# selftok-team/SelftokTokenizer

Measured on NVIDIA B200. Metric: images/sec encode+50-step decode, 256x256/512-tok, higher is better.
Workload: dtype fp16 (IEEE-half operands on tcgen05, fp32 accumulate; encoder/VQ/tables fp32)

## Files before the change

selftoktokenizer_b200/build.py:

```python
from __future__ import annotations

import os
import subprocess
import sys
from concurrent.futures import ThreadPoolExecutor

CSRC = os.path.join(os.path.dirname(os.path.abspath(__file__)), "csrc")
LIB = os.path.join(CSRC, "libselftok_b200.so")
SOURCES = ["kernels_simt.cu", "gemm_tc.cu", "attn_tc5.cu", "engine.cu", "vae.cu"]
HEADERS = ["common.cuh", "kernels.h", os.path.join("..", "..", "include", "selftok_b200.h")]
NVCC_FLAGS = ["-gencode", "arch=compute_100a,code=sm_100a", "-O3", "-lineinfo", "-std=c++17",
              "-Xcompiler", "-fPIC", "-Xcompiler", "-fvisibility=hidden", "--expt-relaxed-constexpr"]


def _nvcc() -> str:
    for c in (os.environ.get("NVCC"), "/usr/local/cuda/bin/nvcc", "nvcc"):
        if c and (os.path.isabs(c) and os.path.exists(c) or not os.path.isabs(c)):
            return c
    raise RuntimeError("nvcc not found")


def needs_build() -> bool:
    if not os.path.exists(LIB):
        return True
    t = os.path.getmtime(LIB)
    deps = [os.path.join(CSRC, f) for f in SOURCES + HEADERS]
    return any(os.path.getmtime(d) > t for d in deps)


def build(force: bool = False, verbose: bool = False) -> str:
    if not force and not needs_build():
        return LIB
    nvcc = _nvcc()
# ... 27 lines not shown
```

selftoktokenizer_b200/csrc/attn_tc5.cu:

```cuda
#include "common.cuh"
#include "kernels.h"

#include <cuda.h>

#include <algorithm>
#include <cstdlib>

namespace stk {

int make_tensor_map_2d(CUtensorMap* map, const void* ptr, uint64_t rows, uint64_t cols, uint32_t box_rows, uint32_t box_cols,
                       int fp16);

namespace {

constexpr int HD = 64, BQ = 128, BKV = 64;
#ifndef SELFTOK_ATTN5_NSB
#define SELFTOK_ATTN5_NSB 2
#endif
constexpr int NSB = SELFTOK_ATTN5_NSB;
#ifndef SELFTOK_ATTN5_SPLIT_ISSUE
#define SELFTOK_ATTN5_SPLIT_ISSUE 0
#endif
constexpr bool SPLIT_ISSUE = SELFTOK_ATTN5_SPLIT_ISSUE != 0;
constexpr int Q_BYTES = BQ * HD * 2, KV_TILE_BYTES = BKV * HD * 2;
constexpr int XCH_BYTES = 6 * BQ * 4;
#ifndef SELFTOK_ATTN5_SPLIT_CTAS
#define SELFTOK_ATTN5_SPLIT_CTAS 2
#endif
template <int NSPLIT> struct A5 {
  static constexpr int PL = NSPLIT == 3 ? 2 : 1;
  static constexpr int MIN_CTAS = NSPLIT == 3 ? SELFTOK_ATTN5_SPLIT_CTAS : 2;
  static constexpr int KV_STAGES = NSPLIT == 3 ? (MIN_CTAS == 2 ? 2 : 3) : 4;
  static constexpr int Q_STAGES = (NSPLIT == 3 && MIN_CTAS == 2) ? 1 : 2;
  static constexpr int Q_STAGE = PL * Q_BYTES;
  static constexpr int KV_STAGE = PL * 2 * KV_TILE_BYTES;
  static constexpr int SMEM_TILES = Q_STAGES * Q_STAGE + KV_STAGES * KV_STAGE;
  static constexpr int SMEM_BYTES = SMEM_TILES + 1024 + 256 + XCH_BYTES;
};
constexpr int TMEM_COLS = 256;
constexpr int NUM_THREADS = 64 + 8 * 32;
constexpr float kRescaleThreshold = 8.0f;

__device__ __forceinline__ uint32_t smem_u32(const void* p) { return (uint32_t)__cvta_generic_to_shared(p); }
__device__ __forceinline__ void mbar_init(uint32_t bar, uint32_t count) {
  asm volatile("mbarrier.init.shared::cta.b64 [%0], %1;" ::"r"(bar), "r"(count) : "memory");
}
__device__ __forceinline__ void mbar_expect_tx(uint32_t bar, uint32_t bytes) {
  asm volatile("mbarrier.arrive.expect_tx.shared::cta.b64 _, [%0], %1;" ::"r"(bar), "r"(bytes) : "memory");
}
__device__ __forceinline__ void mbar_arrive(uint32_t bar) {
  asm volatile("mbarrier.arrive.shared::cta.b64 _, [%0];" ::"r"(bar) : "memory");
}
constexpr uint32_t kSuspendHintNs = 20000;
__device__ __forceinline__ bool mbar_try_wait(uint32_t bar, uint32_t parity) {
  uint32_t ok;
  asm volatile(
      "{\n\t.reg .pred p;\n\t"
      "mbarrier.try_wait.parity.shared::cta.b64 p, [%1], %2, %3;\n\t"
      "selp.u32 %0, 1, 0, p;\n\t}"
      : "=r"(ok) : "r"(bar), "r"(parity), "r"(kSuspendHintNs) : "memory");
  return ok != 0;
}
__device__ __forceinline__ bool mbar_test(uint32_t bar, uint32_t parity) {
  uint32_t ok;
  asm volatile(
      "{\n\t.reg .pred p;\n\t"
      "mbarrier.test_wait.parity.shared::cta.b64 p, [%1], %2;\n\t"
      "selp.u32 %0, 1, 0, p;\n\t}"
      : "=r"(ok) : "r"(bar), "r"(parity) : "memory");
  return ok != 0;
}
__device__ __forceinline__ void mbar_wait(uint32_t bar, uint32_t parity) {
  if (mbar_try_wait(bar, parity)) return;
  const long long t0 = clock64();
  uint32_t spins = 0;
  while (!mbar_try_wait(bar, parity)) {
    if ((++spins & 0x3ff) == 0 && clock64() - t0 > 8000000000LL) {
      printf("selftok attn_tc5: mbarrier timeout (block %d,%d,%d thread %d bar %u parity %u)\n", blockIdx.x, blockIdx.y, blockIdx.z,
             threadIdx.x, bar, parity);
      __trap();
    }
  }
}
__device__ __forceinline__ void tma_load_2d(uint32_t dst, const CUtensorMap* map, uint32_t bar, int c0, int c1) {
  asm volatile(
      "cp.async.bulk.tensor.2d.shared::cluster.global.mbarrier::complete_tx::bytes [%0], [%1, {%3, %4}], [%2];"
      ::"r"(dst), "l"(reinterpret_cast<uint64_t>(map)), "r"(bar), "r"(c0), "r"(c1) : "memory");
}
__device__ __forceinline__ void tc_fence_before() { asm volatile("tcgen05.fence::before_thread_sync;" ::: "memory"); }
__device__ __forceinline__ void tc_fence_after() { asm volatile("tcgen05.fence::after_thread_sync;" ::: "memory"); }
__device__ __forceinline__ void tc_commit(uint32_t bar) {
  asm volatile("tcgen05.commit.cta_group::1.mbarrier::arrive::one.shared::cluster.b64 [%0];" ::"r"(bar) : "memory");
}
__device__ __forceinline__ void tc_mma_f16(uint32_t d_tmem, uint64_t a_desc, uint64_t b_desc, uint32_t idesc, uint32_t accumulate) {
  asm volatile(
      "{\n\t.reg .pred p;\n\t"
      "setp.ne.b32 p, %4, 0;\n\t"
      "tcgen05.mma.cta_group::1.kind::f16 [%0], %1, %2, %3, p;\n\t}"
      ::"r"(d_tmem), "l"(a_desc), "l"(b_desc), "r"(idesc), "r"(accumulate) : "memory");
}
__device__ __forceinline__ void tc_mma_f16_ts(uint32_t d_tmem, uint32_t a_tmem, uint64_t b_desc, uint32_t idesc, uint32_t accumulate) {
  asm volatile(
      "{\n\t.reg .pred p;\n\t"
      "setp.ne.b32 p, %4, 0;\n\t"
      "tcgen05.mma.cta_group::1.kind::f16 [%0], [%1], %2, %3, p;\n\t}"
      ::"r"(d_tmem), "r"(a_tmem), "l"(b_desc), "r"(idesc), "r"(accumulate) : "memory");
}
__device__ __forceinline__ void tmem_ld32(uint32_t taddr, uint32_t (&r)[32]) {
  asm volatile(
      "tcgen05.ld.sync.aligned.32x32b.x32.b32 "
      "{%0, %1, %2, %3, %4, %5, %6, %7, %8, %9, %10, %11, %12, %13, %14, %15, "
      "%16, %17, %18, %19, %20, %21, %22, %23, %24, %25, %26, %27, %28, %29, %30, %31}, [%32];"
      : "=r"(r[0]), "=r"(r[1]), "=r"(r[2]), "=r"(r[3]), "=r"(r[4]), "=r"(r[5]), "=r"(r[6]), "=r"(r[7]),
        "=r"(r[8]), "=r"(r[9]), "=r"(r[10]), "=r"(r[11]), "=r"(r[12]), "=r"(r[13]), "=r"(r[14]), "=r"(r[15]),
        "=r"(r[16]), "=r"(r[17]), "=r"(r[18]), "=r"(r[19]), "=r"(r[20]), "=r"(r[21]), "=r"(r[22]), "=r"(r[23]),
        "=r"(r[24]), "=r"(r[25]), "=r"(r[26]), "=r"(r[27]), "=r"(r[28]), "=r"(r[29]), "=r"(r[30]), "=r"(r[31])
      : "r"(taddr) : "memory");
}
__device__ __forceinline__ void tmem_st32(uint32_t taddr, const uint32_t (&r)[32]) {
  asm volatile(
      "tcgen05.st.sync.aligned.32x32b.x32.b32 [%0], "
      "{%1, %2, %3, %4, %5, %6, %7, %8, %9, %10, %11, %12, %13, %14, %15, %16, "
      "%17, %18, %19, %20, %21, %22, %23, %24, %25, %26, %27, %28, %29, %30, %31, %32};"
      ::"r"(taddr), "r"(r[0]), "r"(r[1]), "r"(r[2]), "r"(r[3]), "r"(r[4]), "r"(r[5]), "r"(r[6]), "r"(r[7]),
        "r"(r[8]), "r"(r[9]), "r"(r[10]), "r"(r[11]), "r"(r[12]), "r"(r[13]), "r"(r[14]), "r"(r[15]),
        "r"(r[16]), "r"(r[17]), "r"(r[18]), "r"(r[19]), "r"(r[20]), "r"(r[21]), "r"(r[22]), "r"(r[23]),
        "r"(r[24]), "r"(r[25]), "r"(r[26]), "r"(r[27]), "r"(r[28]), "r"(r[29]), "r"(r[30]), "r"(r[31])
      : "memory");
}
__device__ __forceinline__ void tmem_st16(uint32_t taddr, const uint32_t (&r)[16]) {
  asm volatile(
      "tcgen05.st.sync.aligned.32x32b.x16.b32 [%0], "
      "{%1, %2, %3, %4, %5, %6, %7, %8, %9, %10, %11, %12, %13, %14, %15, %16};"
      ::"r"(taddr), "r"(r[0]), "r"(r[1]), "r"(r[2]), "r"(r[3]), "r"(r[4]), "r"(r[5]), "r"(r[6]), "r"(r[7]),
        "r"(r[8]), "r"(r[9]), "r"(r[10]), "r"(r[11]), "r"(r[12]), "r"(r[13]), "r"(r[14]), "r"(r[15])
      : "memory");
}
__device__ __forceinline__ void tmem_ld_wait() { asm volatile("tcgen05.wait::ld.sync.aligned;" ::: "memory"); }
__device__ __forceinline__ void tmem_st_wait() { asm volatile("tcgen05.wait::st.sync.aligned;" ::: "memory"); }

__device__ __forceinline__ uint64_t make_smem_desc(uint32_t smem_addr) {
  uint64_t d = 0;
  d |= (uint64_t)((smem_addr >> 4) & 0x3FFF);
  d |= (uint64_t)1 << 16;
  d |= (uint64_t)(1024 >> 4) << 32;
  d |= (uint64_t)1 << 46;
  d |= (uint64_t)2 << 61;
  return d;
}
__device__ __forceinline__ uint32_t make_idesc(int m, int n, int fp16, int b_mn_major) {
  const uint32_t fmt = fp16 ? 0u : 1u;
  return (1u << 4) | (fmt << 7) | (fmt << 10) | ((uint32_t)b_mn_major << 16) | ((uint32_t)(n >> 3) << 17) | ((uint32_t)(m >> 4) << 24);
}

__device__ __forceinline__ float ex2_approx(float x) {
  float y;
  asm("ex2.approx.ftz.f32 %0, %1;" : "=f"(y) : "f"(x));
  return y;
}
__device__ __forceinline__ void scale_sub2(uint32_t s0, uint32_t s1, float scale, float nsub, float& x0, float& x1) {
  asm("{\n\t.reg .b64 x, sc, sb;\n\t"
      "mov.b64 x, {%2, %3};\n\t"
      "mov.b64 sc, {%4, %4};\n\t"
      "mov.b64 sb, {%5, %5};\n\t"
      "fma.rn.f32x2 x, x, sc, sb;\n\t"
      "mov.b64 {%0, %1}, x;\n\t}"
      : "=f"(x0), "=f"(x1) : "r"(s0), "r"(s1), "f"(scale), "f"(nsub));
}
__device__ __forceinline__ void add2(float& a0, float& a1, float e0, float e1) {
  asm("{\n\t.reg .b64 a, b;\n\t"
      "mov.b64 a, {%0, %1};\n\t"
      "mov.b64 b, {%2, %3};\n\t"
      "add.f32x2 a, a, b;\n\t"
      "mov.b64 {%0, %1}, a;\n\t}"
      : "+f"(a0), "+f"(a1) : "f"(e0), "f"(e1));
}
__device__ __forceinline__ uint32_t pack2_16(float lo, float hi, bool fp16) {
  uint32_t r;
  if (fp16) asm("cvt.rn.f16x2.f32 %0, %1, %2;" : "=r"(r) : "f"(hi), "f"(lo));
  else asm("cvt.rn.bf16x2.f32 %0, %1, %2;" : "=r"(r) : "f"(hi), "f"(lo));
  return r;
}

struct Attn5Params {
  AttnOut out;
  int B, S, H, ctx_rows, ctx_keys, fp16;
  float scale_log2e;
};

template <bool FP16, int NSPLIT>
__global__ void __launch_bounds__(NUM_THREADS, A5<NSPLIT>::MIN_CTAS)
attention_tc5_kernel(const __grid_constant__ CUtensorMap map_q, const __grid_constant__ CUtensorMap map_kv,
                     const __grid_constant__ CUtensorMap map_q_lo, const __grid_constant__ CUtensorMap map_kv_lo, const Attn5Params p) {
  static_assert(NSPLIT == 1 || (NSPLIT == 3 && !FP16), "split mode uses bf16 planes");
  using C = A5<NSPLIT>;
  constexpr int KV_STAGES = C::KV_STAGES;
  extern __shared__ uint8_t smem_raw[];
  const uint32_t base = (smem_u32(smem_raw) + 1023u) & ~1023u;
  const uint32_t q_s = base;
  constexpr int QS = C::Q_STAGES;
  static_assert(!SPLIT_ISSUE || QS == 2, "the two-issuer experiment prefetches Q one item ahead");
  const uint32_t kv_s = base + QS * C::Q_STAGE;
  const uint32_t bars = kv_s + KV_STAGES * C::KV_STAGE;
  auto q_full = [&](int qb) { return bars + 8u * qb; };
  auto q_empty = [&](int qb) { return bars + 16 + 8u * qb; };
  auto p_ready = [&](int pb) { return bars + 32 + 8u * pb; };
// ... 282 lines not shown
      }
    }
    if (pend_item >= 0) epilogue(pend_item, n - 1, pend_g, pend_l);
  }
  tc_fence_before();
  __syncthreads();
  if (warp == 2) {
    tc_fence_after();
    asm volatile("tcgen05.dealloc.cta_group::1.sync.aligned.b32 %0, %1;" ::"r"(tmem_base), "r"((uint32_t)TMEM_COLS) : "memory");
  }
}

int g_num_sms_dev[64];
bool g_attr_dev[64];

}

int launch_attention_tc5(const __nv_bfloat16* qkv16, int B, int S, int H, int ctx_rows, int ctx_keys, const AttnOut& out,
                         cudaStream_t s, int fp16, const __nv_bfloat16* qkv_lo) {
  STK_CHECK(qkv16 && B > 0 && S > 0 && H > 0, -1, "attention_tc5: bad arguments");
  STK_CHECK(out.ld % 8 == 0, -1, "attention_tc5: output pitch must be a multiple of 8");
  STK_CHECK(ctx_keys <= S && ctx_rows <= S && ctx_keys >= 0 && ctx_rows >= 0, -1, "attention_tc5: context limits exceed the sequence");
  STK_CHECK(!(fp16 && qkv_lo), -1, "attention_tc5: the split mode uses bf16 planes");
  STK_TRY(gemm_tc_init());
  int dev = 0;
  STK_CUDA(cudaGetDevice(&dev));
  STK_CHECK(dev >= 0 && dev < 64, -1, "attention_tc5: device ordinal out of range");
  if (!g_attr_dev[dev]) {
    STK_CUDA(cudaDeviceGetAttribute(&g_num_sms_dev[dev], cudaDevAttrMultiProcessorCount, dev));
    STK_CUDA(cudaFuncSetAttribute(attention_tc5_kernel<true, 1>, cudaFuncAttributeMaxDynamicSharedMemorySize, A5<1>::SMEM_BYTES));
    STK_CUDA(cudaFuncSetAttribute(attention_tc5_kernel<false, 1>, cudaFuncAttributeMaxDynamicSharedMemorySize, A5<1>::SMEM_BYTES));
    STK_CUDA(cudaFuncSetAttribute(attention_tc5_kernel<false, 3>, cudaFuncAttributeMaxDynamicSharedMemorySize, A5<3>::SMEM_BYTES));
    g_attr_dev[dev] = true;
  }
  const int g_num_sms = g_num_sms_dev[dev];
  CUtensorMap mq, mkv, mql, mkvl;
  const uint64_t rows = (uint64_t)B * S, cols = (uint64_t)3 * H * HD;
  STK_TRY(make_tensor_map_2d(&mq, qkv16, rows, cols, BQ, HD, fp16));
  STK_TRY(make_tensor_map_2d(&mkv, qkv16, rows, cols, BKV, HD, fp16));
  mql = mq; mkvl = mkv;
  if (qkv_lo) {
    STK_TRY(make_tensor_map_2d(&mql, qkv_lo, rows, cols, BQ, HD, 0));
    STK_TRY(make_tensor_map_2d(&mkvl, qkv_lo, rows, cols, BKV, HD, 0));
  }
  Attn5Params p{out, B, S, H, ctx_rows, ctx_keys, fp16, 0.125f * 1.4426950408889634f};
  const int n_items = ((S + BQ - 1) / BQ) * H * B;
  if (qkv_lo) {
    dim3 grid(std::min(n_items, A5<3>::MIN_CTAS * g_num_sms));
    attention_tc5_kernel<false, 3><<<grid, NUM_THREADS, A5<3>::SMEM_BYTES, s>>>(mq, mkv, mql, mkvl, p);
  } else {
    static const int ctas_per_sm = [] { const char* e = getenv("SELFTOK_ATTN5_CTAS_PER_SM"); return (e && e[0] == '1') ? 1 : 2; }();
    dim3 grid(std::min(n_items, ctas_per_sm * g_num_sms));
    if (fp16) attention_tc5_kernel<true, 1><<<grid, NUM_THREADS, A5<1>::SMEM_BYTES, s>>>(mq, mkv, mql, mkvl, p);
    else attention_tc5_kernel<false, 1><<<grid, NUM_THREADS, A5<1>::SMEM_BYTES, s>>>(mq, mkv, mql, mkvl, p);
  }
  count_launch();
  STK_CUDA(cudaGetLastError());
  return 0;
}

}
```

selftoktokenizer_b200/csrc/kernels.h:

```cpp
#pragma once
#include <cuda_runtime.h>
#include <cuda_bf16.h>
#include <stdint.h>

namespace stk {

enum EpiMode { EPI_STORE = 0, EPI_RESID = 1, EPI_SPLIT = 2 };
struct Epilogue {
  int mode = EPI_STORE;
  int act = 0;
  const float* bias = nullptr;
  float* out = nullptr;
  int64_t ldo = 0;
  const float* resid = nullptr;
  const float* gate = nullptr;
  int64_t gate_ld = 0;
  int gate_period = 1;
  const float* addtab = nullptr;
  int64_t add_ld = 0;
  int add_period = 1;
  __nv_bfloat16* out_hi = nullptr;
  __nv_bfloat16* out_lo = nullptr;
  int rpb_in = 0, rpb_out = 0, row_off = 0;
  int fp16 = 0;
// ... 36 lines not shown
int launch_unpatchify_axpy(const float* o, const float* x_in, float* x_out, float dt, int B, int C, int g, int p,
                           cudaStream_t s, const float* o_u = nullptr, float cfg_scale = 1.f);
int launch_transpose(const float* in, float* out, int rows, int cols, cudaStream_t s);
int launch_split_bf16(const float* in, __nv_bfloat16* hi, __nv_bfloat16* lo, int64_t n, cudaStream_t s, int fp16 = 0);
int launch_bcast_rows(const float* src, const float* add, float* out, int B, int64_t rows, int64_t cols, cudaStream_t s);
int launch_crop_pos(const float* pos, float* out, int max_size, int g, int D, cudaStream_t s);
int launch_copy_rows(const float* src, int64_t src_bs, float* dst, int64_t dst_bs, int B, int64_t n_per_batch, cudaStream_t s);

int launch_gemm_tc(const __nv_bfloat16* A_hi, const __nv_bfloat16* A_lo, const __nv_bfloat16* W_hi,
                   const __nv_bfloat16* W_lo, int64_t M, int N, int K, int nsplit, const Epilogue& ep,
                   cudaStream_t s, int fp16 = 0);
struct TcProblem {
  const __nv_bfloat16* A_hi; const __nv_bfloat16* A_lo; const __nv_bfloat16* W_hi; const __nv_bfloat16* W_lo;
  int64_t M; int N; int K;
  Epilogue ep;
  int conv_C = 0, conv_H = 0, conv_W = 0, conv_stride = 1;
};
int launch_gemm_tc_grouped(const TcProblem* probs, int n, int nsplit, cudaStream_t s, int fp16 = 0);
int gemm_tc_init();
void gemm_tc_set_ctas(int n);

int launch_attention_tc5(const __nv_bfloat16* qkv16, int B, int S, int H, int ctx_rows, int ctx_keys, const AttnOut& out,
                         cudaStream_t s, int fp16, const __nv_bfloat16* qkv_lo = nullptr);

}
```

Measured before the change: 21.25.

## Add persistent ping-pong attention kernel with 128-key tiles for non-split path

Adds a new persistent tcgen05 attention kernel that runs two softmax warpgroups in ping-pong over paired query tiles, with 128-wide KV tiles, a 3-stage KV pipeline and a full 512-column TMEM allocation. The single-plane fp16/bf16 path now dispatches to it, and the old NSPLIT=1 variant is dropped. Shared device helpers move into a common header. The aim is to overlap QK/PV MMAs with softmax and to reuse each K/V load across two query tiles, at the cost of one CTA per SM and more complex barrier scheduling.

```diff
diff --git a/selftoktokenizer_b200/build.py b/selftoktokenizer_b200/build.py
--- a/selftoktokenizer_b200/build.py
+++ b/selftoktokenizer_b200/build.py
@@ -7,8 +7,8 @@
 
 CSRC = os.path.join(os.path.dirname(os.path.abspath(__file__)), "csrc")
 LIB = os.path.join(CSRC, "libselftok_b200.so")
-SOURCES = ["kernels_simt.cu", "gemm_tc.cu", "attn_tc5.cu", "engine.cu", "vae.cu"]
-HEADERS = ["common.cuh", "kernels.h", os.path.join("..", "..", "include", "selftok_b200.h")]
+SOURCES = ["kernels_simt.cu", "gemm_tc.cu", "attn_tc5.cu", "attn_pp.cu", "engine.cu", "vae.cu"]
+HEADERS = ["common.cuh", "attn_common.cuh", "kernels.h", os.path.join("..", "..", "include", "selftok_b200.h")]
 NVCC_FLAGS = ["-gencode", "arch=compute_100a,code=sm_100a", "-O3", "-lineinfo", "-std=c++17",
               "-Xcompiler", "-fPIC", "-Xcompiler", "-fvisibility=hidden", "--expt-relaxed-constexpr"]
 
diff --git a/selftoktokenizer_b200/csrc/attn_common.cuh b/selftoktokenizer_b200/csrc/attn_common.cuh
--- /dev/null
+++ b/selftoktokenizer_b200/csrc/attn_common.cuh
@@ -0,0 +1,156 @@
+#pragma once
+#include "common.cuh"
+
+#include <cuda.h>
+
+namespace stk {
+namespace attn {
+
+__device__ __forceinline__ uint32_t smem_u32(const void* p) { return (uint32_t)__cvta_generic_to_shared(p); }
+__device__ __forceinline__ void mbar_init(uint32_t bar, uint32_t count) {
+  asm volatile("mbarrier.init.shared::cta.b64 [%0], %1;" ::"r"(bar), "r"(count) : "memory");
+}
+__device__ __forceinline__ void mbar_expect_tx(uint32_t bar, uint32_t bytes) {
+  asm volatile("mbarrier.arrive.expect_tx.shared::cta.b64 _, [%0], %1;" ::"r"(bar), "r"(bytes) : "memory");
+}
+__device__ __forceinline__ void mbar_arrive(uint32_t bar) {
+  asm volatile("mbarrier.arrive.shared::cta.b64 _, [%0];" ::"r"(bar) : "memory");
+}
+constexpr uint32_t kSuspendHintNs = 20000;
+__device__ __forceinline__ bool mbar_try_wait(uint32_t bar, uint32_t parity) {
+  uint32_t ok;
+  asm volatile(
+      "{\n\t.reg .pred p;\n\t"
+      "mbarrier.try_wait.parity.shared::cta.b64 p, [%1], %2, %3;\n\t"
+      "selp.u32 %0, 1, 0, p;\n\t}"
+      : "=r"(ok) : "r"(bar), "r"(parity), "r"(kSuspendHintNs) : "memory");
+  return ok != 0;
+}
+__device__ __forceinline__ bool mbar_test(uint32_t bar, uint32_t parity) {
+  uint32_t ok;
+  asm volatile(
+      "{\n\t.reg .pred p;\n\t"
+      "mbarrier.test_wait.parity.shared::cta.b64 p, [%1], %2;\n\t"
+      "selp.u32 %0, 1, 0, p;\n\t}"
+      : "=r"(ok) : "r"(bar), "r"(parity) : "memory");
+  return ok != 0;
+}
+__device__ __forceinline__ void mbar_wait(uint32_t bar, uint32_t parity) {
+  if (mbar_try_wait(bar, parity)) return;
+  const long long t0 = clock64();
+  uint32_t spins = 0;
+  while (!mbar_try_wait(bar, parity)) {
+    if ((++spins & 0x3ff) == 0 && clock64() - t0 > 8000000000LL) {
+      printf("selftok attention: mbarrier timeout (block %d,%d,%d thread %d bar %u parity %u)\n", blockIdx.x, blockIdx.y, blockIdx.z,
+             threadIdx.x, bar, parity);
+      __trap();
+    }
+  }
+}
+__device__ __forceinline__ void tma_load_2d(uint32_t dst, const CUtensorMap* map, uint32_t bar, int c0, int c1) {
+  asm volatile(
+      "cp.async.bulk.tensor.2d.shared::cluster.global.mbarrier::complete_tx::bytes [%0], [%1, {%3, %4}], [%2];"
+      ::"r"(dst), "l"(reinterpret_cast<uint64_t>(map)), "r"(bar), "r"(c0), "r"(c1) : "memory");
+}
+__device__ __forceinline__ void tc_fence_before() { asm volatile("tcgen05.fence::before_thread_sync;" ::: "memory"); }
+__device__ __forceinline__ void tc_fence_after() { asm volatile("tcgen05.fence::after_thread_sync;" ::: "memory"); }
+__device__ __forceinline__ void tc_commit(uint32_t bar) {
+  asm volatile("tcgen05.commit.cta_group::1.mbarrier::arrive::one.shared::cluster.b64 [%0];" ::"r"(bar) : "memory");
+}
+__device__ __forceinline__ void tc_mma_f16(uint32_t d_tmem, uint64_t a_desc, uint64_t b_desc, uint32_t idesc, uint32_t accumulate) {
+  asm volatile(
+      "{\n\t.reg .pred p;\n\t"
+      "setp.ne.b32 p, %4, 0;\n\t"
+      "tcgen05.mma.cta_group::1.kind::f16 [%0], %1, %2, %3, p;\n\t}"
+      ::"r"(d_tmem), "l"(a_desc), "l"(b_desc), "r"(idesc), "r"(accumulate) : "memory");
+}
+__device__ __forceinline__ void tc_mma_f16_ts(uint32_t d_tmem, uint32_t a_tmem, uint64_t b_desc, uint32_t idesc, uint32_t accumulate) {
+  asm volatile(
+      "{\n\t.reg .pred p;\n\t"
+      "setp.ne.b32 p, %4, 0;\n\t"
+      "tcgen05.mma.cta_group::1.kind::f16 [%0], [%1], %2, %3, p;\n\t}"
+      ::"r"(d_tmem), "r"(a_tmem), "l"(b_desc), "r"(idesc), "r"(accumulate) : "memory");
+}
+__device__ __forceinline__ void tmem_ld32(uint32_t taddr, uint32_t (&r)[32]) {
+  asm volatile(
+      "tcgen05.ld.sync.aligned.32x32b.x32.b32 "
+      "{%0, %1, %2, %3, %4, %5, %6, %7, %8, %9, %10, %11, %12, %13, %14, %15, "
+      "%16, %17, %18, %19, %20, %21, %22, %23, %24, %25, %26, %27, %28, %29, %30, %31}, [%32];"
+      : "=r"(r[0]), "=r"(r[1]), "=r"(r[2]), "=r"(r[3]), "=r"(r[4]), "=r"(r[5]), "=r"(r[6]), "=r"(r[7]),
+        "=r"(r[8]), "=r"(r[9]), "=r"(r[10]), "=r"(r[11]), "=r"(r[12]), "=r"(r[13]), "=r"(r[14]), "=r"(r[15]),
+        "=r"(r[16]), "=r"(r[17]), "=r"(r[18]), "=r"(r[19]), "=r"(r[20]), "=r"(r[21]), "=r"(r[22]), "=r"(r[23]),
+        "=r"(r[24]), "=r"(r[25]), "=r"(r[26]), "=r"(r[27]), "=r"(r[28]), "=r"(r[29]), "=r"(r[30]), "=r"(r[31])
+      : "r"(taddr) : "memory");
+}
+__device__ __forceinline__ void tmem_st32(uint32_t taddr, const uint32_t (&r)[32]) {
+  asm volatile(
+      "tcgen05.st.sync.aligned.32x32b.x32.b32 [%0], "
+      "{%1, %2, %3, %4, %5, %6, %7, %8, %9, %10, %11, %12, %13, %14, %15, %16, "
+      "%17, %18, %19, %20, %21, %22, %23, %24, %25, %26, %27, %28, %29, %30, %31, %32};"
+      ::"r"(taddr), "r"(r[0]), "r"(r[1]), "r"(r[2]), "r"(r[3]), "r"(r[4]), "r"(r[5]), "r"(r[6]), "r"(r[7]),
+        "r"(r[8]), "r"(r[9]), "r"(r[10]), "r"(r[11]), "r"(r[12]), "r"(r[13]), "r"(r[14]), "r"(r[15]),
+        "r"(r[16]), "r"(r[17]), "r"(r[18]), "r"(r[19]), "r"(r[20]), "r"(r[21]), "r"(r[22]), "r"(r[23]),
+        "r"(r[24]), "r"(r[25]), "r"(r[26]), "r"(r[27]), "r"(r[28]), "r"(r[29]), "r"(r[30]), "r"(r[31])
+      : "memory");
+}
+__device__ __forceinline__ void tmem_st16(uint32_t taddr, const uint32_t (&r)[16]) {
+  asm volatile(
+      "tcgen05.st.sync.aligned.32x32b.x16.b32 [%0], "
+      "{%1, %2, %3, %4, %5, %6, %7, %8, %9, %10, %11, %12, %13, %14, %15, %16};"
+      ::"r"(taddr), "r"(r[0]), "r"(r[1]), "r"(r[2]), "r"(r[3]), "r"(r[4]), "r"(r[5]), "r"(r[6]), "r"(r[7]),
+        "r"(r[8]), "r"(r[9]), "r"(r[10]), "r"(r[11]), "r"(r[12]), "r"(r[13]), "r"(r[14]), "r"(r[15])
+      : "memory");
+}
+__device__ __forceinline__ void tmem_ld_wait() { asm volatile("tcgen05.wait::ld.sync.aligned;" ::: "memory"); }
+__device__ __forceinline__ void tmem_st_wait() { asm volatile("tcgen05.wait::st.sync.aligned;" ::: "memory"); }
+
+__device__ __forceinline__ uint64_t make_smem_desc(uint32_t smem_addr) {
+  uint64_t d = 0;
+  d |= (uint64_t)((smem_addr >> 4) & 0x3FFF);
+  d |= (uint64_t)1 << 16;
+  d |= (uint64_t)(1024 >> 4) << 32;
+  d |= (uint64_t)1 << 46;
+  d |= (uint64_t)2 << 61;
+  return d;
+}
+__device__ __forceinline__ uint32_t make_idesc(int m, int n, int fp16, int b_mn_major) {
+  const uint32_t fmt = fp16 ? 0u : 1u;
+  return (1u << 4) | (fmt << 7) | (fmt << 10) | ((uint32_t)b_mn_major << 16) | ((uint32_t)(n >> 3) << 17) | ((uint32_t)(m >> 4) << 24);
+}
+
+__device__ __forceinline__ float max3(float a, float b, float c) {
+  float d;
+  asm("max.f32 %0, %1, %2, %3;" : "=f"(d) : "f"(a), "f"(b), "f"(c));
+  return d;
+}
+__device__ __forceinline__ float ex2_approx(float x) {
+  float y;
+  asm("ex2.approx.ftz.f32 %0, %1;" : "=f"(y) : "f"(x));
+  return y;
+}
+__device__ __forceinline__ void scale_sub2(uint32_t s0, uint32_t s1, float scale, float nsub, float& x0, float& x1) {
+  asm("{\n\t.reg .b64 x, sc, sb;\n\t"
+      "mov.b64 x, {%2, %3};\n\t"
+      "mov.b64 sc, {%4, %4};\n\t"
+      "mov.b64 sb, {%5, %5};\n\t"
+      "fma.rn.f32x2 x, x, sc, sb;\n\t"
+      "mov.b64 {%0, %1}, x;\n\t}"
+      : "=f"(x0), "=f"(x1) : "r"(s0), "r"(s1), "f"(scale), "f"(nsub));
+}
+__device__ __forceinline__ void add2(float& a0, float& a1, float e0, float e1) {
+  asm("{\n\t.reg .b64 a, b;\n\t"
+      "mov.b64 a, {%0, %1};\n\t"
+      "mov.b64 b, {%2, %3};\n\t"
+      "add.f32x2 a, a, b;\n\t"
+      "mov.b64 {%0, %1}, a;\n\t}"
+      : "+f"(a0), "+f"(a1) : "f"(e0), "f"(e1));
+}
+__device__ __forceinline__ uint32_t pack2_16(float lo, float hi, bool fp16) {
+  uint32_t r;
+  if (fp16) asm("cvt.rn.f16x2.f32 %0, %1, %2;" : "=r"(r) : "f"(hi), "f"(lo));
+  else asm("cvt.rn.bf16x2.f32 %0, %1, %2;" : "=r"(r) : "f"(hi), "f"(lo));
+  return r;
+}
+
+}
+}
diff --git a/selftoktokenizer_b200/csrc/attn_pp.cu b/selftoktokenizer_b200/csrc/attn_pp.cu
--- /dev/null
+++ b/selftoktokenizer_b200/csrc/attn_pp.cu
@@ -0,0 +1,376 @@
+#include "attn_common.cuh"
+#include "common.cuh"
+#include "kernels.h"
+
+#include <cuda.h>
+
+#include <algorithm>
+
+namespace stk {
+
+int make_tensor_map_2d(CUtensorMap* map, const void* ptr, uint64_t rows, uint64_t cols, uint32_t box_rows, uint32_t box_cols,
+                       int fp16);
+
+namespace {
+
+using namespace attn;
+
+constexpr int HD = 64, BQ = 128, BKV = 128, KV_STAGES = 3;
+constexpr int TILE_BYTES = 128 * HD * 2;
+constexpr int Q_STAGE = 2 * TILE_BYTES;
+constexpr int KV_STAGE = 2 * TILE_BYTES;
+constexpr int SMEM_BYTES = 2 * Q_STAGE + KV_STAGES * KV_STAGE + 1024 + 256;
+constexpr int TMEM_COLS = 512;
+constexpr int NUM_THREADS = 10 * 32;
+constexpr int MAX_REGS = 168;
+constexpr float kRescaleThreshold = 8.0f;
+
+struct PpParams {
+  AttnOut out;
+  int B, S, H, ctx_rows, ctx_keys;
+  int qpi;
+  float scale_log2e;
+};
+
+struct Item {
+  int b, h, qt0, nqt;
+  int nkt, klast;
+};
+__device__ __forceinline__ Item item_info(const PpParams& p, int nq, int npi, int item) {
+  Item it;
+  const int pi = item % npi;
+  it.h = (item / npi) % p.H;
+  it.b = item / (npi * p.H);
+  it.qt0 = pi * p.qpi;
+  it.nqt = min(p.qpi, nq - it.qt0);
+  const int kmax = ((it.qt0 + it.nqt) * BQ <= p.ctx_rows) ? p.ctx_keys : p.S;
+  it.nkt = (kmax + BKV - 1) / BKV;
+  it.klast = kmax - (it.nkt - 1) * BKV;
+  return it;
+}
+
+struct Op { int item, n, j, t, g; Item it; };
+__device__ __forceinline__ Op op_first(const PpParams& p, int nq, int npi, int n_items) {
+  Op o{(int)blockIdx.x, 0, 0, 0, 0, {}};
+  if (o.item < n_items) o.it = item_info(p, nq, npi, o.item);
+  return o;
+}
+__device__ __forceinline__ void op_next(Op& o, const PpParams& p, int nq, int npi, int n_items, bool pair) {
+  if (++o.t < (pair ? o.it.nqt : 1)) return;
+  o.t = 0; ++o.g;
+  if (++o.j < o.it.nkt) return;
+  o.j = 0; ++o.n; o.item += gridDim.x;
+  if (o.item < n_items) o.it = item_info(p, nq, npi, o.item);
+}
+
+template <bool FP16>
+__global__ void __maxnreg__(MAX_REGS)
+attention_pp_kernel(const __grid_constant__ CUtensorMap map, const PpParams p) {
+  extern __shared__ uint8_t smem_raw[];
+  const uint32_t base = (smem_u32(smem_raw) + 1023u) & ~1023u;
+  const uint32_t q_s = base;
+  const uint32_t kv_s = base + 2 * Q_STAGE;
+  const uint32_t bars = kv_s + KV_STAGES * KV_STAGE;
+  auto q_full = [&](int qb) { return bars + 8u * qb; };
+  auto q_empty = [&](int qb) { return bars + 16 + 8u * qb; };
+  auto s_full = [&](int sb) { return bars + 32 + 8u * sb; };
+  auto p_ready = [&](int sb) { return bars + 48 + 8u * sb; };
+  auto pv_done = [&](int sb) { return bars + 64 + 8u * sb; };
+  auto o_done = [&](int t, int ib) { return bars + 80 + 8u * (2 * t + ib); };
+  auto kv_full = [&](int st) { return bars + 112 + 8u * st; };
+  auto kv_empty = [&](int st) { return bars + 112 + 8u * KV_STAGES + 8u * st; };
+  auto tok = [&](int w) { return bars + 112 + 16u * KV_STAGES + 8u * w; };
+  const uint32_t tmem_slot = bars + 128 + 16u * KV_STAGES;
+  uint32_t* tmem_slot_ptr = reinterpret_cast<uint32_t*>(smem_raw + (tmem_slot - smem_u32(smem_raw)));
+
+  const int warp = threadIdx.x >> 5, lane = threadIdx.x & 31;
+  const int S = p.S;
+  const bool pair = p.qpi == 2;
+  const int nq = (S + BQ - 1) / BQ;
+  const int npi = (nq + p.qpi - 1) / p.qpi;
+  const int n_items = npi * p.H * p.B;
+
+  if (warp == 8 && lane == 0) {
+    for (int i = 0; i < 2; ++i) {
+      mbar_init(q_full(i), 1); mbar_init(q_empty(i), 1);
+      mbar_init(s_full(i), 1); mbar_init(p_ready(i), 4); mbar_init(pv_done(i), 1);
+    }
+    for (int i = 0; i < 4; ++i) mbar_init(o_done(i >> 1, i & 1), 1);
+    for (int st = 0; st < KV_STAGES; ++st) { mbar_init(kv_full(st), 1); mbar_init(kv_empty(st), 1); }
+    mbar_init(tok(0), 4); mbar_init(tok(1), 4);
+    asm volatile("fence.mbarrier_init.release.cluster;" ::: "memory");
+  }
+  if (warp == 0) {
+    asm volatile("tcgen05.alloc.cta_group::1.sync.aligned.shared::cta.b32 [%0], %1;" ::"r"(tmem_slot), "r"((uint32_t)TMEM_COLS) : "memory");
+    asm volatile("tcgen05.relinquish_alloc_permit.cta_group::1.sync.aligned;" ::: "memory");
+  }
+  tc_fence_before();
+  __syncthreads();
+  tc_fence_after();
+  const uint32_t tmem_base = *tmem_slot_ptr;
+  auto s_tmem = [&](int sb) { return tmem_base + 128u * sb; };
+  auto o_tmem = [&](int t, int ib) { return tmem_base + 256u + 64u * (2 * t + ib); };
+
+  if (warp == 8) {
+    if (lane == 0) {
+      auto load_q = [&](int item, int n) {
+        const Item it = item_info(p, nq, npi, item);
+        const int qb = n & 1;
+        mbar_wait(q_empty(qb), ((n >> 1) & 1) ^ 1);
+        mbar_expect_tx(q_full(qb), it.nqt * TILE_BYTES);
+        for (int t = 0; t < it.nqt; ++t)
+          tma_load_2d(q_s + qb * Q_STAGE + t * TILE_BYTES, &map, q_full(qb), it.h * HD, it.b * S + (it.qt0 + t) * BQ);
+      };
+      int g = 0, n = 0;
+      if ((int)blockIdx.x < n_items) load_q(blockIdx.x, 0);
+      for (int item = blockIdx.x; item < n_items; item += gridDim.x, ++n) {
+        const Item it = item_info(p, nq, npi, item);
+        if (item + (int)gridDim.x < n_items) load_q(item + gridDim.x, n + 1);
+        for (int j = 0; j < it.nkt; ++j, ++g) {
+          const int st = g % KV_STAGES;
+          mbar_wait(kv_empty(st), ((g / KV_STAGES) & 1) ^ 1);
+          const uint32_t ks = kv_s + st * KV_STAGE;
+          mbar_expect_tx(kv_full(st), KV_STAGE);
+          tma_load_2d(ks, &map, kv_full(st), (p.H + it.h) * HD, it.b * S + j * BKV);
+          tma_load_2d(ks + TILE_BYTES, &map, kv_full(st), (2 * p.H + it.h) * HD, it.b * S + j * BKV);
+        }
+      }
+    }
+  } else if (warp == 9) {
+    if (lane == 0) {
+      Op cq = op_first(p, nq, npi, n_items), cp = cq;
+      auto sbuf = [&](const Op& o) { return pair ? o.t : (o.j & 1); };
+      const uint32_t idesc_pv = make_idesc(BQ, HD, FP16 ? 1 : 0, 1);
+      uint32_t qk_ahead = 0, pv_ph = 0, o_ph = 0;
+      while (cp.item < n_items) {
+        while (cq.item < n_items) {
+          const int sb = sbuf(cq);
+          if (qk_ahead >> sb & 1) break;
+          const int nslot = pair ? cq.it.nqt : 1;
+          const bool last_j = cq.j == cq.it.nkt - 1;
+          if (cq.j == 0 && cq.t == 0) mbar_wait(q_full(cq.n & 1), (cq.n >> 1) & 1);
+          if (cq.t == 0) mbar_wait(kv_full(cq.g % KV_STAGES), (cq.g / KV_STAGES) & 1);
+          tc_fence_after();
+          const uint32_t qs = q_s + (cq.n & 1) * Q_STAGE + cq.t * TILE_BYTES, ks = kv_s + (cq.g % KV_STAGES) * KV_STAGE;
+          const int ncols = last_j ? (cq.it.klast + 31) & ~31 : BKV;
+          const uint32_t idesc_qk = make_idesc(BQ, ncols, FP16 ? 1 : 0, 0);
+#pragma unroll
+          for (int k = 0; k < HD / 16; ++k)
+            tc_mma_f16(s_tmem(sb), make_smem_desc(qs + k * 32), make_smem_desc(ks + k * 32), idesc_qk, k > 0 ? 1u : 0u);
+          tc_commit(s_full(sb));
+          if (last_j && cq.t == nslot - 1) tc_commit(q_empty(cq.n & 1));
+          qk_ahead |= 1u << sb;
+          op_next(cq, p, nq, npi, n_items, pair);
+        }
+        const int sb = sbuf(cp), tq = pair ? cp.t : 0;
+        const bool last_j = cp.j == cp.it.nkt - 1;
+        const int st = cp.g % KV_STAGES;
+        mbar_wait(p_ready(sb), pv_ph >> sb & 1);
+        tc_fence_after();
+        const int nks = last_j ? (cp.it.klast + 15) >> 4 : BKV / 16;
+        const uint32_t vs = kv_s + st * KV_STAGE + TILE_BYTES, od = o_tmem(tq, o_ph >> tq & 1);
+#pragma unroll
+        for (int k = 0; k < BKV / 16; ++k)
+          if (k < nks)
+            tc_mma_f16_ts(od, s_tmem(sb) + 32 * (k >> 1) + 8 * (k & 1), make_smem_desc(vs + k * 2048), idesc_pv, (cp.j > 0 || k > 0) ? 1u : 0u);
+        tc_commit(pv_done(sb));
+        pv_ph ^= 1u << sb;
+        qk_ahead &= ~(1u << sb);
+        if (cp.t == (pair ? cp.it.nqt : 1) - 1) tc_commit(kv_empty(st));
+        if (last_j) { tc_commit(o_done(tq, o_ph >> tq & 1)); o_ph ^= 1u << tq; }
+        op_next(cp, p, nq, npi, n_items, pair);
+      }
+    }
+  } else {
+    const int wg = warp >> 2, quarter = warp & 3;
+    const int rl = quarter * 32 + lane;
+    const uint32_t lane_addr = (uint32_t)(quarter * 32) << 16;
+    auto epilogue = [&](int item, int k, float l_run) {
+      const Item it = item_info(p, nq, npi, item);
+      const int b = it.b, h = it.h, row = (it.qt0 + (pair ? wg : 0)) * BQ + rl;
+      mbar_wait(o_done(wg, k & 1), (k >> 1) & 1);
+      tc_fence_after();
+      uint32_t r0[32], r1[32];
+      tmem_ld32(o_tmem(wg, k & 1) + lane_addr, r0);
+      tmem_ld32(o_tmem(wg, k & 1) + 32 + lane_addr, r1);
+      tmem_ld_wait();
+      if (row < S) {
+        const float inv = 1.0f / l_run;
+        const AttnOut& t = p.out;
+        const bool inA = row < t.split;
+        const int64_t orow = inA ? ((int64_t)b * t.split + row) : ((int64_t)b * (S - t.split) + (row - t.split));
+        float* of = inA ? t.f32_a : t.f32_b;
+        uint16_t* oh = reinterpret_cast<uint16_t*>(inA ? t.hi_a : t.hi_b);
+        uint16_t* ol = reinterpret_cast<uint16_t*>(inA ? t.lo_a : t.lo_b);
+        const int64_t o = orow * t.ld + (int64_t)h * HD;
+#pragma unroll
+        for (int c = 0; c < 8; ++c) {
+          float y[8];
+#pragma unroll
+          for (int q = 0; q < 8; ++q) y[q] = __uint_as_float(c < 4 ? r0[c * 8 + q] : r1[(c - 4) * 8 + q]) * inv;
+          if (of) {
+            *reinterpret_cast<float4*>(of + o + c * 8) = make_float4(y[0], y[1], y[2], y[3]);
+            *reinterpret_cast<float4*>(of + o + c * 8 + 4) = make_float4(y[4], y[5], y[6], y[7]);
+          }
+          if (oh) {
+            uint32_t hp[4];
+#pragma unroll
+            for (int q = 0; q < 4; ++q) hp[q] = pack2_sat16(y[2 * q], y[2 * q + 1], FP16);
+            *reinterpret_cast<uint4*>(oh + o + c * 8) = make_uint4(hp[0], hp[1], hp[2], hp[3]);
+            if (!FP16 && ol) {
+              uint32_t lp[4];
+#pragma unroll
+              for (int q = 0; q < 4; ++q) lp[q] = pack2_resid_bf16(y[2 * q], y[2 * q + 1], hp[q]);
+              *reinterpret_cast<uint4*>(ol + o + c * 8) = make_uint4(lp[0], lp[1], lp[2], lp[3]);
+            }
+          }
+        }
+      }
+    };
+    uint32_t ph = 0;
+    int k_items = 0;
+    int m_pair = 0;
+    int pend_item = -1;
+    float pend_l = 1.f;
+    for (int item = blockIdx.x; item < n_items; item += gridDim.x) {
+      const Item it = item_info(p, nq, npi, item);
+      if (wg >= (pair ? it.nqt : 1)) continue;
+      const int row = (it.qt0 + (pair ? wg : 0)) * BQ + rl;
+      const int kmax = (row < p.ctx_rows) ? p.ctx_keys : S;
+      float m_run = -INFINITY, l_run = 0.f;
+      for (int j = 0; j < it.nkt; ++j) {
+        const int sb = pair ? wg : (j & 1);
+        const int nch = j == it.nkt - 1 ? (it.klast + 31) >> 5 : BKV / 32;
+        mbar_wait(s_full(sb), ph >> sb & 1);
+        tc_fence_after();
+        uint32_t r[4][32];
+#pragma unroll
+        for (int c = 0; c < 4; ++c) tmem_ld32(s_tmem(sb) + 32 * c + lane_addr, r[c]);
+        tmem_ld_wait();
+        const int k0 = j * BKV;
+        if (k0 + BKV > kmax) {
+#pragma unroll
+          for (int c = 0; c < 4; ++c)
+#pragma unroll
+            for (int i = 0; i < 32; ++i)
+              if (k0 + 32 * c + i >= kmax) r[c][i] = 0xff800000u;
+        }
+        float ma = -INFINITY, mb = -INFINITY;
+#pragma unroll
+        for (int c = 0; c < 4; ++c)
+          if (c < nch) {
+#pragma unroll
+            for (int i = 0; i < 32; i += 4) {
+              ma = max3(ma, __uint_as_float(r[c][i]), __uint_as_float(r[c][i + 1]));
+              mb = max3(mb, __uint_as_float(r[c][i + 2]), __uint_as_float(r[c][i + 3]));
+            }
+          }
+        float m_new = fmaxf(m_run, fmaxf(ma, mb) * p.scale_log2e);
+        if (m_new - m_run <= kRescaleThreshold) m_new = m_run;
+        const float sub = (m_new == -INFINITY) ? 0.f : m_new;
+        const float corr = (m_new == m_run || m_new == -INFINITY) ? 1.f : ex2_approx(m_run - m_new);
+        const bool handoff = pair && it.nqt == 2;
+        if (handoff && (wg == 1 || m_pair > 0)) mbar_wait(tok(wg), (wg == 1 ? m_pair : m_pair - 1) & 1);
+        float rsp[4] = {0.f, 0.f, 0.f, 0.f};
+        const float nsub = -sub;
+#pragma unroll
+        for (int c = 0; c < 4; ++c)
+          if (c < nch) {
+            uint32_t w[16];
+#pragma unroll
+            for (int q = 0; q < 16; ++q) {
+              float x0, x1;
+              scale_sub2(r[c][2 * q], r[c][2 * q + 1], p.scale_log2e, nsub, x0, x1);
+              const float e0 = ex2_approx(x0), e1 = ex2_approx(x1);
+              add2(rsp[2 * (q & 1)], rsp[2 * (q & 1) + 1], e0, e1);
+              w[q] = pack2_16(e0, e1, FP16);
+            }
+            tmem_st16(s_tmem(sb) + 32 * c + lane_addr, w);
+          }
+        if (handoff) {
+          __syncwarp();
+          if (lane == 0) mbar_arrive(tok(wg ^ 1));
+          ++m_pair;
+        }
+        l_run = l_run * corr + ((rsp[0] + rsp[1]) + (rsp[2] + rsp[3]));
+        m_run = m_new;
+        if (j > 0 && !__all_sync(0xffffffffu, corr == 1.0f)) {
+          const int sp = pair ? sb : ((j - 1) & 1);
+          mbar_wait(pv_done(sp), (ph >> sp & 1) ^ 1);
+          tc_fence_after();
+          const uint32_t od = o_tmem(wg, k_items & 1) + lane_addr;
+          tmem_ld32(od, r[0]);
+          tmem_ld32(od + 32, r[1]);
+          tmem_ld_wait();
+#pragma unroll
+          for (int i = 0; i < 32; ++i) {
+            r[0][i] = __float_as_uint(__uint_as_float(r[0][i]) * corr);
+            r[1][i] = __float_as_uint(__uint_as_float(r[1][i]) * corr);
+          }
+          tmem_st32(od, r[0]);
+          tmem_st32(od + 32, r[1]);
+        }
+        tmem_st_wait();
+        tc_fence_before();
+        __syncwarp();
+        if (lane == 0) mbar_arrive(p_ready(sb));
+        ph ^= 1u << sb;
+        if (j == 0 && pend_item >= 0) {
+          epilogue(pend_item, k_items - 1, pend_l);
+          pend_item = -1;
+        }
+      }
+      pend_item = item;
+      pend_l = l_run;
+      ++k_items;
+    }
+    if (pend_item >= 0) epilogue(pend_item, k_items - 1, pend_l);
+  }
+  tc_fence_before();
+  __syncthreads();
+  if (warp == 0) {
+    tc_fence_after();
+    asm volatile("tcgen05.dealloc.cta_group::1.sync.aligned.b32 %0, %1;" ::"r"(tmem_base), "r"((uint32_t)TMEM_COLS) : "memory");
+  }
+}
+
+int g_num_sms_dev[64];
+bool g_attr_dev[64];
+
+}
+
+int launch_attention_pp(const __nv_bfloat16* qkv16, int B, int S, int H, int ctx_rows, int ctx_keys, const AttnOut& out,
+                        cudaStream_t s, int fp16) {
+  STK_CHECK(qkv16 && B > 0 && S > 0 && H > 0, -1, "attention_pp: bad arguments");
+  STK_CHECK(out.ld % 8 == 0, -1, "attention_pp: output pitch must be a multiple of 8");
+  STK_CHECK(ctx_keys <= S && ctx_rows <= S && ctx_keys >= 0 && ctx_rows >= 0, -1, "attention_pp: context limits exceed the sequence");
+  STK_CHECK(ctx_rows == 0 || ctx_keys > 0, -1, "attention_pp: context rows need at least one visible key");
+  STK_TRY(gemm_tc_init());
+  int dev = 0;
+  STK_CUDA(cudaGetDevice(&dev));
+  STK_CHECK(dev >= 0 && dev < 64, -1, "attention_pp: device ordinal out of range");
+  if (!g_attr_dev[dev]) {
+    STK_CUDA(cudaDeviceGetAttribute(&g_num_sms_dev[dev], cudaDevAttrMultiProcessorCount, dev));
+    STK_CUDA(cudaFuncSetAttribute(attention_pp_kernel<true>, cudaFuncAttributeMaxDynamicSharedMemorySize, SMEM_BYTES));
+    STK_CUDA(cudaFuncSetAttribute(attention_pp_kernel<false>, cudaFuncAttributeMaxDynamicSharedMemorySize, SMEM_BYTES));
+    g_attr_dev[dev] = true;
+  }
+  const int num_sms = g_num_sms_dev[dev];
+  CUtensorMap map;
+  STK_TRY(make_tensor_map_2d(&map, qkv16, (uint64_t)B * S, (uint64_t)3 * H * HD, 128, HD, fp16));
+  const int nq = (S + BQ - 1) / BQ;
+  PpParams p{out, B, S, H, ctx_rows, ctx_keys, 2, 0.125f * 1.4426950408889634f};
+  int n_items = ((nq + 1) / 2) * H * B;
+  if (n_items < num_sms) {
+    p.qpi = 1;
+    n_items = nq * H * B;
+  }
+  dim3 grid(std::min(n_items, num_sms));
+  if (fp16) attention_pp_kernel<true><<<grid, NUM_THREADS, SMEM_BYTES, s>>>(map, p);
+  else attention_pp_kernel<false><<<grid, NUM_THREADS, SMEM_BYTES, s>>>(map, p);
+  count_launch();
+  STK_CUDA(cudaGetLastError());
+  return 0;
+}
+
+}
diff --git a/selftoktokenizer_b200/csrc/attn_tc5.cu b/selftoktokenizer_b200/csrc/attn_tc5.cu
--- a/selftoktokenizer_b200/csrc/attn_tc5.cu
+++ b/selftoktokenizer_b200/csrc/attn_tc5.cu
@@ -1,10 +1,10 @@
+#include "attn_common.cuh"
 #include "common.cuh"
 #include "kernels.h"
 
 #include <cuda.h>
 
 #include <algorithm>
-#include <cstdlib>
 
 namespace stk {
 
@@ -12,6 +12,8 @@
                        int fp16);
 
 namespace {
+
+using namespace attn;
 
 constexpr int HD = 64, BQ = 128, BKV = 64;
 #ifndef SELFTOK_ATTN5_NSB
@@ -41,147 +43,6 @@
 constexpr int NUM_THREADS = 64 + 8 * 32;
 constexpr float kRescaleThreshold = 8.0f;
 
-__device__ __forceinline__ uint32_t smem_u32(const void* p) { return (uint32_t)__cvta_generic_to_shared(p); }
-__device__ __forceinline__ void mbar_init(uint32_t bar, uint32_t count) {
-  asm volatile("mbarrier.init.shared::cta.b64 [%0], %1;" ::"r"(bar), "r"(count) : "memory");
-}
-__device__ __forceinline__ void mbar_expect_tx(uint32_t bar, uint32_t bytes) {
-  asm volatile("mbarrier.arrive.expect_tx.shared::cta.b64 _, [%0], %1;" ::"r"(bar), "r"(bytes) : "memory");
-}
-__device__ __forceinline__ void mbar_arrive(uint32_t bar) {
-  asm volatile("mbarrier.arrive.shared::cta.b64 _, [%0];" ::"r"(bar) : "memory");
-}
-constexpr uint32_t kSuspendHintNs = 20000;
-__device__ __forceinline__ bool mbar_try_wait(uint32_t bar, uint32_t parity) {
-  uint32_t ok;
-  asm volatile(
-      "{\n\t.reg .pred p;\n\t"
-      "mbarrier.try_wait.parity.shared::cta.b64 p, [%1], %2, %3;\n\t"
-      "selp.u32 %0, 1, 0, p;\n\t}"
-      : "=r"(ok) : "r"(bar), "r"(parity), "r"(kSuspendHintNs) : "memory");
-  return ok != 0;
-}
-__device__ __forceinline__ bool mbar_test(uint32_t bar, uint32_t parity) {
-  uint32_t ok;
-  asm volatile(
-      "{\n\t.reg .pred p;\n\t"
-      "mbarrier.test_wait.parity.shared::cta.b64 p, [%1], %2;\n\t"
-      "selp.u32 %0, 1, 0, p;\n\t}"
-      : "=r"(ok) : "r"(bar), "r"(parity) : "memory");
-  return ok != 0;
-}
-__device__ __forceinline__ void mbar_wait(uint32_t bar, uint32_t parity) {
-  if (mbar_try_wait(bar, parity)) return;
-  const long long t0 = clock64();
-  uint32_t spins = 0;
-  while (!mbar_try_wait(bar, parity)) {
-    if ((++spins & 0x3ff) == 0 && clock64() - t0 > 8000000000LL) {
-      printf("selftok attn_tc5: mbarrier timeout (block %d,%d,%d thread %d bar %u parity %u)\n", blockIdx.x, blockIdx.y, blockIdx.z,
-             threadIdx.x, bar, parity);
-      __trap();
-    }
-  }
-}
-__device__ __forceinline__ void tma_load_2d(uint32_t dst, const CUtensorMap* map, uint32_t bar, int c0, int c1) {
-  asm volatile(
-      "cp.async.bulk.tensor.2d.shared::cluster.global.mbarrier::complete_tx::bytes [%0], [%1, {%3, %4}], [%2];"
-      ::"r"(dst), "l"(reinterpret_cast<uint64_t>(map)), "r"(bar), "r"(c0), "r"(c1) : "memory");
-}
-__device__ __forceinline__ void tc_fence_before() { asm volatile("tcgen05.fence::before_thread_sync;" ::: "memory"); }
-__device__ __forceinline__ void tc_fence_after() { asm volatile("tcgen05.fence::after_thread_sync;" ::: "memory"); }
-__device__ __forceinline__ void tc_commit(uint32_t bar) {
-  asm volatile("tcgen05.commit.cta_group::1.mbarrier::arrive::one.shared::cluster.b64 [%0];" ::"r"(bar) : "memory");
-}
-__device__ __forceinline__ void tc_mma_f16(uint32_t d_tmem, uint64_t a_desc, uint64_t b_desc, uint32_t idesc, uint32_t accumulate) {
-  asm volatile(
-      "{\n\t.reg .pred p;\n\t"
-      "setp.ne.b32 p, %4, 0;\n\t"
-      "tcgen05.mma.cta_group::1.kind::f16 [%0], %1, %2, %3, p;\n\t}"
-      ::"r"(d_tmem), "l"(a_desc), "l"(b_desc), "r"(idesc), "r"(accumulate) : "memory");
-}
-__device__ __forceinline__ void tc_mma_f16_ts(uint32_t d_tmem, uint32_t a_tmem, uint64_t b_desc, uint32_t idesc, uint32_t accumulate) {
-  asm volatile(
-      "{\n\t.reg .pred p;\n\t"
-      "setp.ne.b32 p, %4, 0;\n\t"
-      "tcgen05.mma.cta_group::1.kind::f16 [%0], [%1], %2, %3, p;\n\t}"
-      ::"r"(d_tmem), "r"(a_tmem), "l"(b_desc), "r"(idesc), "r"(accumulate) : "memory");
-}
-__device__ __forceinline__ void tmem_ld32(uint32_t taddr, uint32_t (&r)[32]) {
-  asm volatile(
-      "tcgen05.ld.sync.aligned.32x32b.x32.b32 "
-      "{%0, %1, %2, %3, %4, %5, %6, %7, %8, %9, %10, %11, %12, %13, %14, %15, "
-      "%16, %17, %18, %19, %20, %21, %22, %23, %24, %25, %26, %27, %28, %29, %30, %31}, [%32];"
-      : "=r"(r[0]), "=r"(r[1]), "=r"(r[2]), "=r"(r[3]), "=r"(r[4]), "=r"(r[5]), "=r"(r[6]), "=r"(r[7]),
-        "=r"(r[8]), "=r"(r[9]), "=r"(r[10]), "=r"(r[11]), "=r"(r[12]), "=r"(r[13]), "=r"(r[14]), "=r"(r[15]),
-        "=r"(r[16]), "=r"(r[17]), "=r"(r[18]), "=r"(r[19]), "=r"(r[20]), "=r"(r[21]), "=r"(r[22]), "=r"(r[23]),
-        "=r"(r[24]), "=r"(r[25]), "=r"(r[26]), "=r"(r[27]), "=r"(r[28]), "=r"(r[29]), "=r"(r[30]), "=r"(r[31])
-      : "r"(taddr) : "memory");
-}
-__device__ __forceinline__ void tmem_st32(uint32_t taddr, const uint32_t (&r)[32]) {
-  asm volatile(
-      "tcgen05.st.sync.aligned.32x32b.x32.b32 [%0], "
-      "{%1, %2, %3, %4, %5, %6, %7, %8, %9, %10, %11, %12, %13, %14, %15, %16, "
-      "%17, %18, %19, %20, %21, %22, %23, %24, %25, %26, %27, %28, %29, %30, %31, %32};"
-      ::"r"(taddr), "r"(r[0]), "r"(r[1]), "r"(r[2]), "r"(r[3]), "r"(r[4]), "r"(r[5]), "r"(r[6]), "r"(r[7]),
-        "r"(r[8]), "r"(r[9]), "r"(r[10]), "r"(r[11]), "r"(r[12]), "r"(r[13]), "r"(r[14]), "r"(r[15]),
-        "r"(r[16]), "r"(r[17]), "r"(r[18]), "r"(r[19]), "r"(r[20]), "r"(r[21]), "r"(r[22]), "r"(r[23]),
-        "r"(r[24]), "r"(r[25]), "r"(r[26]), "r"(r[27]), "r"(r[28]), "r"(r[29]), "r"(r[30]), "r"(r[31])
-      : "memory");
-}
-__device__ __forceinline__ void tmem_st16(uint32_t taddr, const uint32_t (&r)[16]) {
-  asm volatile(
-      "tcgen05.st.sync.aligned.32x32b.x16.b32 [%0], "
-      "{%1, %2, %3, %4, %5, %6, %7, %8, %9, %10, %11, %12, %13, %14, %15, %16};"
-      ::"r"(taddr), "r"(r[0]), "r"(r[1]), "r"(r[2]), "r"(r[3]), "r"(r[4]), "r"(r[5]), "r"(r[6]), "r"(r[7]),
-        "r"(r[8]), "r"(r[9]), "r"(r[10]), "r"(r[11]), "r"(r[12]), "r"(r[13]), "r"(r[14]), "r"(r[15])
-      : "memory");
-}
-__device__ __forceinline__ void tmem_ld_wait() { asm volatile("tcgen05.wait::ld.sync.aligned;" ::: "memory"); }
-__device__ __forceinline__ void tmem_st_wait() { asm volatile("tcgen05.wait::st.sync.aligned;" ::: "memory"); }
-
-__device__ __forceinline__ uint64_t make_smem_desc(uint32_t smem_addr) {
-  uint64_t d = 0;
-  d |= (uint64_t)((smem_addr >> 4) & 0x3FFF);
-  d |= (uint64_t)1 << 16;
-  d |= (uint64_t)(1024 >> 4) << 32;
-  d |= (uint64_t)1 << 46;
-  d |= (uint64_t)2 << 61;
-  return d;
-}
-__device__ __forceinline__ uint32_t make_idesc(int m, int n, int fp16, int b_mn_major) {
-  const uint32_t fmt = fp16 ? 0u : 1u;
-  return (1u << 4) | (fmt << 7) | (fmt << 10) | ((uint32_t)b_mn_major << 16) | ((uint32_t)(n >> 3) << 17) | ((uint32_t)(m >> 4) << 24);
-}
-
-__device__ __forceinline__ float ex2_approx(float x) {
-  float y;
-  asm("ex2.approx.ftz.f32 %0, %1;" : "=f"(y) : "f"(x));
-  return y;
-}
-__device__ __forceinline__ void scale_sub2(uint32_t s0, uint32_t s1, float scale, float nsub, float& x0, float& x1) {
-  asm("{\n\t.reg .b64 x, sc, sb;\n\t"
-      "mov.b64 x, {%2, %3};\n\t"
-      "mov.b64 sc, {%4, %4};\n\t"
-      "mov.b64 sb, {%5, %5};\n\t"
-      "fma.rn.f32x2 x, x, sc, sb;\n\t"
-      "mov.b64 {%0, %1}, x;\n\t}"
-      : "=f"(x0), "=f"(x1) : "r"(s0), "r"(s1), "f"(scale), "f"(nsub));
-}
-__device__ __forceinline__ void add2(float& a0, float& a1, float e0, float e1) {
-  asm("{\n\t.reg .b64 a, b;\n\t"
-      "mov.b64 a, {%0, %1};\n\t"
-      "mov.b64 b, {%2, %3};\n\t"
-      "add.f32x2 a, a, b;\n\t"
-      "mov.b64 {%0, %1}, a;\n\t}"
-      : "+f"(a0), "+f"(a1) : "f"(e0), "f"(e1));
-}
-__device__ __forceinline__ uint32_t pack2_16(float lo, float hi, bool fp16) {
-  uint32_t r;
-  if (fp16) asm("cvt.rn.f16x2.f32 %0, %1, %2;" : "=r"(r) : "f"(hi), "f"(lo));
-  else asm("cvt.rn.bf16x2.f32 %0, %1, %2;" : "=r"(r) : "f"(hi), "f"(lo));
-  return r;
-}
-
 struct Attn5Params {
   AttnOut out;
   int B, S, H, ctx_rows, ctx_keys, fp16;
@@ -510,14 +371,13 @@
   STK_CHECK(out.ld % 8 == 0, -1, "attention_tc5: output pitch must be a multiple of 8");
   STK_CHECK(ctx_keys <= S && ctx_rows <= S && ctx_keys >= 0 && ctx_rows >= 0, -1, "attention_tc5: context limits exceed the sequence");
   STK_CHECK(!(fp16 && qkv_lo), -1, "attention_tc5: the split mode uses bf16 planes");
+  if (!qkv_lo) return launch_attention_pp(qkv16, B, S, H, ctx_rows, ctx_keys, out, s, fp16);
   STK_TRY(gemm_tc_init());
   int dev = 0;
   STK_CUDA(cudaGetDevice(&dev));
   STK_CHECK(dev >= 0 && dev < 64, -1, "attention_tc5: device ordinal out of range");
   if (!g_attr_dev[dev]) {
     STK_CUDA(cudaDeviceGetAttribute(&g_num_sms_dev[dev], cudaDevAttrMultiProcessorCount, dev));
-    STK_CUDA(cudaFuncSetAttribute(attention_tc5_kernel<true, 1>, cudaFuncAttributeMaxDynamicSharedMemorySize, A5<1>::SMEM_BYTES));
-    STK_CUDA(cudaFuncSetAttribute(attention_tc5_kernel<false, 1>, cudaFuncAttributeMaxDynamicSharedMemorySize, A5<1>::SMEM_BYTES));
     STK_CUDA(cudaFuncSetAttribute(attention_tc5_kernel<false, 3>, cudaFuncAttributeMaxDynamicSharedMemorySize, A5<3>::SMEM_BYTES));
     g_attr_dev[dev] = true;
   }
@@ -526,22 +386,12 @@
   const uint64_t rows = (uint64_t)B * S, cols = (uint64_t)3 * H * HD;
   STK_TRY(make_tensor_map_2d(&mq, qkv16, rows, cols, BQ, HD, fp16));
   STK_TRY(make_tensor_map_2d(&mkv, qkv16, rows, cols, BKV, HD, fp16));
-  mql = mq; mkvl = mkv;
-  if (qkv_lo) {
-    STK_TRY(make_tensor_map_2d(&mql, qkv_lo, rows, cols, BQ, HD, 0));
-    STK_TRY(make_tensor_map_2d(&mkvl, qkv_lo, rows, cols, BKV, HD, 0));
-  }
+  STK_TRY(make_tensor_map_2d(&mql, qkv_lo, rows, cols, BQ, HD, 0));
+  STK_TRY(make_tensor_map_2d(&mkvl, qkv_lo, rows, cols, BKV, HD, 0));
   Attn5Params p{out, B, S, H, ctx_rows, ctx_keys, fp16, 0.125f * 1.4426950408889634f};
   const int n_items = ((S + BQ - 1) / BQ) * H * B;
-  if (qkv_lo) {
-    dim3 grid(std::min(n_items, A5<3>::MIN_CTAS * g_num_sms));
-    attention_tc5_kernel<false, 3><<<grid, NUM_THREADS, A5<3>::SMEM_BYTES, s>>>(mq, mkv, mql, mkvl, p);
-  } else {
-    static const int ctas_per_sm = [] { const char* e = getenv("SELFTOK_ATTN5_CTAS_PER_SM"); return (e && e[0] == '1') ? 1 : 2; }();
-    dim3 grid(std::min(n_items, ctas_per_sm * g_num_sms));
-    if (fp16) attention_tc5_kernel<true, 1><<<grid, NUM_THREADS, A5<1>::SMEM_BYTES, s>>>(mq, mkv, mql, mkvl, p);
-    else attention_tc5_kernel<false, 1><<<grid, NUM_THREADS, A5<1>::SMEM_BYTES, s>>>(mq, mkv, mql, mkvl, p);
-  }
+  dim3 grid(std::min(n_items, A5<3>::MIN_CTAS * g_num_sms));
+  attention_tc5_kernel<false, 3><<<grid, NUM_THREADS, A5<3>::SMEM_BYTES, s>>>(mq, mkv, mql, mkvl, p);
   count_launch();
   STK_CUDA(cudaGetLastError());
   return 0;
diff --git a/selftoktokenizer_b200/csrc/kernels.h b/selftoktokenizer_b200/csrc/kernels.h
--- a/selftoktokenizer_b200/csrc/kernels.h
+++ b/selftoktokenizer_b200/csrc/kernels.h
@@ -82,5 +82,7 @@
 
 int launch_attention_tc5(const __nv_bfloat16* qkv16, int B, int S, int H, int ctx_rows, int ctx_keys, const AttnOut& out,
                          cudaStream_t s, int fp16, const __nv_bfloat16* qkv_lo = nullptr);
+int launch_attention_pp(const __nv_bfloat16* qkv16, int B, int S, int H, int ctx_rows, int ctx_keys, const AttnOut& out,
+                        cudaStream_t s, int fp16);
 
 }
```

Result: slower. 20.82, median of 6 (-2.0%).
